# somanshu25/GPU-Accelerated-Point-Cloud-Registration-Using-Hierarchical-GMM

Hardware: AMD Instinct MI355X
Metric: EM iterations/sec (N points x J components); E-step achieved HBM GB/s (higher is better)
Workload: dtype f32; 1 GPU; BASELINE configs[2]/[4]: uniform [0,1)^3 cloud, N=1,000,000 pts per GPU (seed=rank), flat diag GMM J=800 (flavour W), fused device-resident EM, tol=0; N>1: frames are shards of one joint fit, all-reduce of (7J+2) f64 sufficient statistics per iteration; points_per_gpu=1000000, components=800, cov_type=diag, device= (gfx950:sramecc+:xnack-), compute_units=256

## Files before the change

### gpu-accelerated-point-cloud-registration-using-hierarchical-gmm_amd/csrc/flat_fused_body.h

```cpp
    constexpr int K = NSLOT;
    constexpr int KP = K / 2;
    constexpr bool ODD = (K & 1) != 0;
    const int lane = lane_id();
    f2 mu0[KP + 1], mu1[KP + 1], mu2[KP + 1], g0[KP + 1], g1[KP + 1], g2[KP + 1], cc[KP + 1];
    f2 s0[KP + 1], a0[KP + 1], a1[KP + 1], a2[KP + 1], b0[KP + 1], b1[KP + 1], b2[KP + 1];
    float mu0s = 0.f, mu1s = 0.f, mu2s = 0.f, g0s = 0.f, g1s = 0.f, g2s = 0.f, cs = NEG_INF;
    float s0s = 0.f, a0s = 0.f, a1s = 0.f, a2s = 0.f, b0s = 0.f, b1s = 0.f, b2s = 0.f;
#pragma unroll
    for (int p = 0; p < KP; ++p) {
        const int ja = (2 * p) * 64 + lane, jb = (2 * p + 1) * 64 + lane;
        mu0[p] = f2{pack[(PK_MU + 0) * Jpad + ja], pack[(PK_MU + 0) * Jpad + jb]};
        mu1[p] = f2{pack[(PK_MU + 1) * Jpad + ja], pack[(PK_MU + 1) * Jpad + jb]};
        mu2[p] = f2{pack[(PK_MU + 2) * Jpad + ja], pack[(PK_MU + 2) * Jpad + jb]};
        g0[p] = f2{pack[(PK_G + 0) * Jpad + ja], pack[(PK_G + 0) * Jpad + jb]};
        g1[p] = f2{pack[(PK_G + 1) * Jpad + ja], pack[(PK_G + 1) * Jpad + jb]};
        g2[p] = f2{pack[(PK_G + 2) * Jpad + ja], pack[(PK_G + 2) * Jpad + jb]};
        cc[p] = f2{pack[PK_C * Jpad + ja], pack[PK_C * Jpad + jb]};
        s0[p] = a0[p] = a1[p] = a2[p] = b0[p] = b1[p] = b2[p] = f2{0.f, 0.f};
    }
    if (ODD) {
        const int j = (K - 1) * 64 + lane;
        mu0s = pack[(PK_MU + 0) * Jpad + j]; mu1s = pack[(PK_MU + 1) * Jpad + j]; mu2s = pack[(PK_MU + 2) * Jpad + j];
        g0s = pack[(PK_G + 0) * Jpad + j]; g1s = pack[(PK_G + 1) * Jpad + j]; g2s = pack[(PK_G + 2) * Jpad + j];
        cs = pack[PK_C * Jpad + j];
    }

    float m0 = cs;
#pragma unroll
    for (int p = 0; p < KP; ++p) m0 = fmaxf(m0, fmaxf(cc[p].x, cc[p].y));
    m0 = wave_max_dpp(m0);
    const bool small_shift = allow_const_shift && m0 <= CS_MAX_SHIFT && m0 >= -64.0f;

    int64_t r0;
    int nrows;
    FLAT_FUSED_ROW_RANGE(n, r0, nrows);
    const float* const xw = X + 3 * r0;
    double lsum = 0.0;
    float o0 = 0.f, o1 = 0.f, o2 = 0.f, ow = 0.f;
#pragma unroll
    for (int p = 0; p < KP; ++p) {
        const float wa = pack[PK_W * Jpad + (2 * p) * 64 + lane], wb = pack[PK_W * Jpad + (2 * p + 1) * 64 + lane];
        o0 = fmaf(wa, mu0[p].x, fmaf(wb, mu0[p].y, o0));
        o1 = fmaf(wa, mu1[p].x, fmaf(wb, mu1[p].y, o1));
        o2 = fmaf(wa, mu2[p].x, fmaf(wb, mu2[p].y, o2));
        ow += wa + wb;
    }
    if (ODD) {
        const float ws = pack[PK_W * Jpad + (K - 1) * 64 + lane];
        o0 = fmaf(ws, mu0s, o0); o1 = fmaf(ws, mu1s, o1); o2 = fmaf(ws, mu2s, o2);
        ow += ws;
    }
    {
        ow = wave_sum_dpp(ow);
        const float inv_w = ow > 0.f ? 1.0f / ow : 0.f;
        o0 = wave_sum_dpp(o0) * inv_w; o1 = wave_sum_dpp(o1) * inv_w; o2 = wave_sum_dpp(o2) * inv_w;
        if (!(fabsf(o0) < 3.0e38f)) o0 = 0.f;
        if (!(fabsf(o1) < 3.0e38f)) o1 = 0.f;
        if (!(fabsf(o2) < 3.0e38f)) o2 = 0.f;
    }
    auto rows = [&](auto cs_tag) {
    constexpr bool CS = decltype(cs_tag)::value;
    if (CS) {
        const f2 M0 = f2{m0, m0};
#pragma unroll
        for (int p = 0; p < KP; ++p) cc[p] = cc[p] - M0;
        cs -= m0;
    }
    const float eps_scale = __builtin_amdgcn_exp2f(-m0);
    float eps_v = FLAT_EPS;
    asm volatile("" : "+v"(eps_v));
    float lacc = 0.f;
    float x0 = 0.f, x1 = 0.f, x2 = 0.f;
    float sw = 1.f;
    double swsum = 0.0;
    if (nrows > 0) { x0 = xw[0]; x1 = xw[1]; x2 = xw[2]; if (WEIGHTED) sw = SW[r0]; }
    for (int row = 0; row < nrows; ++row) {
        const int nrow = (row + 1 < nrows) ? row + 1 : row;
        const float* xn = xw + 3 * (int64_t)nrow;
        const float nx0 = xn[0], nx1 = xn[1], nx2 = xn[2];
        float nsw = 1.f;
        if constexpr (WEIGHTED) nsw = SW[r0 + nrow];
        if (!WEIGHTED || !weight_is_zero(sw)) {
            const f2 X0 = f2{x0, x0}, X1 = f2{x1, x1}, X2 = f2{x2, x2};
            const float xo0 = x0 - o0, xo1 = x1 - o1, xo2 = x2 - o2;
            const f2 XO0 = f2{xo0, xo0}, XO1 = f2{xo1, xo1}, XO2 = f2{xo2, xo2};

            f2 wl[KP + 1];
            f2 q0[KP + 1], q1[KP + 1], q2[KP + 1];
            float q0s = 0.f, q1s = 0.f, q2s = 0.f;
            float wls = NEG_INF;
            float m = NEG_INF;
            f2 sacc = f2{0.f, 0.f};
#pragma unroll
            for (int p = 0; p < KP; ++p) {
                const f2 d0 = X0 - mu0[p], d1 = X1 - mu1[p], d2 = X2 - mu2[p];
                q0[p] = d0 * d0; q1[p] = d1 * d1; q2[p] = d2 * d2;
                f2 a = cc[p] - g0[p] * q0[p];
                a = a - g1[p] * q1[p];
                a = a - g2[p] * q2[p];
                if (CS) {
                    wl[p] = f2{__builtin_amdgcn_exp2f(a.x), __builtin_amdgcn_exp2f(a.y)};
                    sacc = p == 0 ? wl[p] : sacc + wl[p];
                } else {
                    wl[p] = a;
                    m = fmaxf(m, fmaxf(a.x, a.y));
                }
            }
            if (ODD) {
                const float d0 = x0 - mu0s, d1 = x1 - mu1s, d2 = x2 - mu2s;
                q0s = d0 * d0; q1s = d1 * d1; q2s = d2 * d2;
                float a = fmaf(-g0s, q0s, cs);
                a = fmaf(-g1s, q1s, a);
                a = fmaf(-g2s, q2s, a);
                wls = CS ? __builtin_amdgcn_exp2f(a) : a;
                m = fmaxf(m, a);
            }
            if (CS) {
                m = m0;
            } else {
                m = wave_max_dpp(m);
                if (m == NEG_INF) m = 0.f;
                const f2 M = f2{m, m};
#pragma unroll
                for (int p = 0; p < KP; ++p) {
                    const f2 t = wl[p] - M;
                    wl[p] = f2{__builtin_amdgcn_exp2f(t.x), __builtin_amdgcn_exp2f(t.y)};
                    sacc = p == 0 ? wl[p] : sacc + wl[p];
                }
                if (ODD) wls = __builtin_amdgcn_exp2f(wls - m);
            }
            float s = sacc.x + sacc.y;
            if (ODD) s += wls;
            s = wave_sum_dpp(s);
            float inv_den;
            if (CS) {
                const float den = fmaf(eps_v, eps_scale, s);
                inv_den = __builtin_amdgcn_rcpf(den);
                if constexpr (WEIGHTED) lacc = fmaf(sw, __builtin_amdgcn_logf(den), lacc);
                else lacc += __builtin_amdgcn_logf(den);
                if constexpr (!WEIGHTED) {
                    if ((row & 7) == 7) {
                        asm volatile("" ::: "memory");
                        lsum += (double)lacc;
                        lacc = 0.f;
                    }
                }
            } else {
                const float lpn2 = lpn2_from(m, s, inv_den);
                if constexpr (WEIGHTED) lsum += (double)sw * (double)(lpn2 * LN2);
                else lsum += (double)(lpn2 * LN2);
            }
            if constexpr (WEIGHTED) inv_den *= sw;
            const f2 INV = f2{inv_den, inv_den};
#pragma unroll
            for (int p = 0; p < KP; ++p) {
                const f2 rr = wl[p] * INV;
                s0[p] += rr;
                a0[p] += rr * XO0; a1[p] += rr * XO1; a2[p] += rr * XO2;
                b0[p] += rr * q0[p]; b1[p] += rr * q1[p]; b2[p] += rr * q2[p];
            }
            if (ODD) {
                const float rr = wls * inv_den;
                s0s += rr;
                a0s = fmaf(rr, xo0, a0s); a1s = fmaf(rr, xo1, a1s); a2s = fmaf(rr, xo2, a2s);
                b0s = fmaf(rr, q0s, b0s); b1s = fmaf(rr, q1s, b1s); b2s = fmaf(rr, q2s, b2s);
            }
        }
        if constexpr (WEIGHTED) {
            if (CS && (row & 7) == 7) {
                asm volatile("" ::: "memory");
                lsum += (double)lacc;
                lacc = 0.f;
            }
        }
        x0 = nx0; x1 = nx1; x2 = nx2;
        if constexpr (WEIGHTED) sw = nsw;
    }
    if constexpr (WEIGHTED) {
        if (CS) {
            for (int64_t i = r0 + lane; i < r0 + nrows; i += 64) swsum += (double)SW[i];
            swsum = wave_sum_f64(swsum);
        }
    }
    if (CS) lsum = (lsum + (double)lacc + (WEIGHTED ? swsum : (double)nrows) * (double)m0) * (double)LN2;
    };
    if (small_shift) rows(std::true_type{});
    else rows(std::false_type{});
    {
        const f2 O0 = f2{o0, o0}, O1 = f2{o1, o1}, O2 = f2{o2, o2};
#pragma unroll
        for (int p = 0; p < KP; ++p) {
            a0[p] -= (mu0[p] - O0) * s0[p]; a1[p] -= (mu1[p] - O1) * s0[p]; a2[p] -= (mu2[p] - O2) * s0[p];
        }
        if (ODD) {
            a0s = fmaf(-(mu0s - o0), s0s, a0s); a1s = fmaf(-(mu1s - o1), s0s, a1s); a2s = fmaf(-(mu2s - o2), s0s, a2s);
        }
    }

    constexpr int ST = NSLOT * 64, STP = ST + 8, CP = FLAT_NSTAT * STP;
    __shared__ float sh[3 * CP];
    __shared__ double shl[WAVES_PER_BLOCK];
    const int w = wave_in_block();
    if (lane == 0) shl[w] = lsum;
    auto put = [&](float* base, int k, bool first, float v0, float v1, float v2, float v3, float v4, float v5, float v6) {
        float* q = base + k * 64 + lane;
        if (first) { q[0 * STP] = v0; q[1 * STP] = v1; q[2 * STP] = v2; q[3 * STP] = v3; q[4 * STP] = v4; q[5 * STP] = v5; q[6 * STP] = v6; }
        else { q[0 * STP] += v0; q[1 * STP] += v1; q[2 * STP] += v2; q[3 * STP] += v3; q[4 * STP] += v4; q[5 * STP] += v5; q[6 * STP] += v6; }
    };
    auto put_all = [&](float* base, bool first) {
#pragma unroll
        for (int p = 0; p < KP; ++p) {
            put(base, 2 * p, first, s0[p].x, a0[p].x, a1[p].x, a2[p].x, b0[p].x, b1[p].x, b2[p].x);
            put(base, 2 * p + 1, first, s0[p].y, a0[p].y, a1[p].y, a2[p].y, b0[p].y, b1[p].y, b2[p].y);
        }
        if (ODD) put(base, K - 1, first, s0s, a0s, a1s, a2s, b0s, b1s, b2s);
    };
    if (w != 1) put_all(sh + (w == 0 ? 0 : w - 1) * CP, true);
    __syncthreads();
    if (w == 1) put_all(sh, false);
    __syncthreads();
    auto total = [&](int i) { return (sh[i] + sh[CP + i]) + sh[2 * CP + i]; };
    if (comp_major) {
        float* outp = partials + (size_t)FLAT_FUSED_BLOCK * FLAT_CM_STRIDE * Jpad;
        for (int idx = threadIdx.x; idx < FLAT_CM_STRIDE * ST; idx += BLOCK) {
            const int j = idx / FLAT_CM_STRIDE, st = idx % FLAT_CM_STRIDE;
            outp[idx] = st < FLAT_NSTAT ? total(st * STP + j) : 0.f;
        }
    } else {
        float* outp = partials + (size_t)FLAT_FUSED_BLOCK * FLAT_NSTAT * Jpad;
        for (int idx = threadIdx.x; idx < FLAT_NSTAT * ST; idx += BLOCK) {
            const int st = idx / ST, j = idx % ST;
            outp[st * Jpad + j] = total(st * STP + j);
        }
    }
    if (threadIdx.x == 0) {
        double t = 0.0;
        for (int i = 0; i < WAVES_PER_BLOCK; ++i) t += shl[i];
        lpn_partials[FLAT_FUSED_BLOCK] = t;
    }
```

### gpu-accelerated-point-cloud-registration-using-hierarchical-gmm_amd/csrc/flat_fused_device.h

```cpp
#pragma once
#include "hgmm_ctx.h"
#include "wave_ops.h"

namespace hgmm {

constexpr float NEG_INF = -__builtin_huge_valf();
constexpr float LOG2E = 1.4426950408889634f;
constexpr float LN2 = 0.6931471805599453f;
constexpr int PK_MU = 0, PK_G = 3, PK_C = 6, PK_W = 7;
constexpr int PK_ROWS = 8;
typedef float f2 __attribute__((ext_vector_type(2)));
constexpr int WAVES_PER_BLOCK = 4;
constexpr int BLOCK = WAVES_PER_BLOCK * 64;

constexpr float CS_MAX_SHIFT = 60.0f;
__device__ __forceinline__ float lpn2_from(float m2, float s, float& inv_den) {
    const bool tiny = m2 < -64.0f;
    const float mc = tiny ? -64.0f : m2;
    const float den = fmaf(FLAT_EPS, __builtin_amdgcn_exp2f(-mc), tiny ? 0.0f : s);
    inv_den = tiny ? 0.0f : __builtin_amdgcn_rcpf(den);
    return mc + __builtin_amdgcn_logf(den);
}

__device__ __forceinline__ void wave_row_range(int64_t n, int64_t& r0, int64_t& r1) {
    const int64_t nw = (int64_t)gridDim.x * WAVES_PER_BLOCK;
    const int64_t gw = (int64_t)blockIdx.x * WAVES_PER_BLOCK + wave_in_block();
    const int64_t per = (n + nw - 1) / nw;
    r0 = gw * per;
    r1 = r0 + per < n ? r0 + per : n;
    if (r0 > n) r0 = n;
}
__device__ __forceinline__ int64_t uniform_i64(int64_t v) {
    const int lo = __builtin_amdgcn_readfirstlane((int)(v & 0xffffffffLL)), hi = __builtin_amdgcn_readfirstlane((int)(v >> 32));
    return ((int64_t)hi << 32) | (int64_t)(unsigned int)lo;
}
__device__ __forceinline__ void wave_row_range_uniform(int64_t n, int64_t& r0, int& nrows) {
    int64_t r1;
    wave_row_range(n, r0, r1);
    r0 = uniform_i64(r0);
    nrows = (int)(uniform_i64(r1) - r0);
}

__device__ __forceinline__ void wave_row_range_uniform(int64_t n, unsigned block, unsigned nblocks, int64_t& r0, int& nrows) {
    const int64_t nw = (int64_t)nblocks * WAVES_PER_BLOCK;
    const int64_t gw = (int64_t)block * WAVES_PER_BLOCK + wave_in_block();
    const int64_t per = (n + nw - 1) / nw;
    int64_t a = gw * per;
    const int64_t b = a + per < n ? a + per : n;
    if (a > n) a = n;
    r0 = uniform_i64(a);
    nrows = (int)(uniform_i64(b) - r0);
}

__device__ __forceinline__ bool weight_is_zero(float s) { return (__float_as_uint(s) & 0x7fffffffu) == 0u; }


template <class T>
__device__ __forceinline__ T* global_ptr(T* p) {
    typedef __attribute__((address_space(1))) T* gptr;
    return (T*)(gptr)(uintptr_t)p;
}
template <class T>
__device__ __forceinline__ const T* constant_ptr(const T* p) {
    typedef __attribute__((address_space(4))) const T* cptr;
    return (const T*)(cptr)(uintptr_t)p;
}


void launch_fused_batch_weighted(int slots, unsigned grid, hipStream_t stream, const FlatBatchMember* members,
                                 const int2* wg_table, int J, int Jpad, int parity);

}
```

Before: 3131 EM it/s (1M-pt x 800-comp frames x iterations per second, all GPUs).

## Unroll fused E-step row loop into double-buffered trips with batched point prefetch

Restructures the per-wave row loop in the fused EM kernel. For slot counts up to 13 in the small-shift path, rows are processed in trips of eight, split into two halves whose point coordinates are prefetched as a batch and held in scalar registers, with sched_barriers fencing the loads. The log-likelihood flush to double happens once per trip instead of through a per-row branch. The aim is to hide point-load latency and cut per-row loop and branch overhead, at the cost of higher register pressure, code size and a remainder loop.

```diff
diff --git a/gpu-accelerated-point-cloud-registration-using-hierarchical-gmm_amd/csrc/flat_fused_body.h b/gpu-accelerated-point-cloud-registration-using-hierarchical-gmm_amd/csrc/flat_fused_body.h
--- a/gpu-accelerated-point-cloud-registration-using-hierarchical-gmm_amd/csrc/flat_fused_body.h
+++ b/gpu-accelerated-point-cloud-registration-using-hierarchical-gmm_amd/csrc/flat_fused_body.h
@@ -70,16 +70,8 @@
     float eps_v = FLAT_EPS;
     asm volatile("" : "+v"(eps_v));
     float lacc = 0.f;
-    float x0 = 0.f, x1 = 0.f, x2 = 0.f;
-    float sw = 1.f;
     double swsum = 0.0;
-    if (nrows > 0) { x0 = xw[0]; x1 = xw[1]; x2 = xw[2]; if (WEIGHTED) sw = SW[r0]; }
-    for (int row = 0; row < nrows; ++row) {
-        const int nrow = (row + 1 < nrows) ? row + 1 : row;
-        const float* xn = xw + 3 * (int64_t)nrow;
-        const float nx0 = xn[0], nx1 = xn[1], nx2 = xn[2];
-        float nsw = 1.f;
-        if constexpr (WEIGHTED) nsw = SW[r0 + nrow];
+    auto row_em = [&](const float x0, const float x1, const float x2, const float sw) __attribute__((always_inline)) {
         if (!WEIGHTED || !weight_is_zero(sw)) {
             const f2 X0 = f2{x0, x0}, X1 = f2{x1, x1}, X2 = f2{x2, x2};
             const float xo0 = x0 - o0, xo1 = x1 - o1, xo2 = x2 - o2;
@@ -138,13 +130,6 @@
                 inv_den = __builtin_amdgcn_rcpf(den);
                 if constexpr (WEIGHTED) lacc = fmaf(sw, __builtin_amdgcn_logf(den), lacc);
                 else lacc += __builtin_amdgcn_logf(den);
-                if constexpr (!WEIGHTED) {
-                    if ((row & 7) == 7) {
-                        asm volatile("" ::: "memory");
-                        lsum += (double)lacc;
-                        lacc = 0.f;
-                    }
-                }
             } else {
                 const float lpn2 = lpn2_from(m, s, inv_den);
                 if constexpr (WEIGHTED) lsum += (double)sw * (double)(lpn2 * LN2);
@@ -161,17 +146,77 @@
             }
             if (ODD) {
                 const float rr = wls * inv_den;
-                s0s += rr;
+                if constexpr (WEIGHTED) s0s += rr;
+                else s0s = fmaf(wls, inv_den, s0s);
                 a0s = fmaf(rr, xo0, a0s); a1s = fmaf(rr, xo1, a1s); a2s = fmaf(rr, xo2, a2s);
                 b0s = fmaf(rr, q0s, b0s); b1s = fmaf(rr, q1s, b1s); b2s = fmaf(rr, q2s, b2s);
             }
         }
-        if constexpr (WEIGHTED) {
-            if (CS && (row & 7) == 7) {
-                asm volatile("" ::: "memory");
-                lsum += (double)lacc;
-                lacc = 0.f;
-            }
+    };
+    constexpr int TRIP = NSLOT <= 13 ? FUSED_TRIP : 1;
+    int row = 0;
+    if constexpr (CS && TRIP > 1) {
+        constexpr int HALF = TRIP > 1 ? TRIP / 2 : 1;
+        static_assert(8 % TRIP == 0, "a flush every eight rows falls at the end of a trip");
+        if (nrows >= TRIP) {
+            float xa[3 * HALF], xb[3 * HALF], wa[HALF], wb[HALF];
+            auto half_trip = [&](const float (&have)[3 * HALF], const float (&whave)[HALF], float (&into)[3 * HALF],
+                                 float (&winto)[HALF], const int next) __attribute__((always_inline)) {
+#pragma unroll
+                for (int t = 0; t < HALF; ++t) {
+                    float c0 = have[3 * t], c1 = have[3 * t + 1], c2 = have[3 * t + 2];
+                    asm volatile("" : "+s"(c0), "+s"(c1), "+s"(c2));
+                    row_em(c0, c1, c2, whave[t]);
+                    if (ODD) asm volatile("" : : "v"(s0s), "v"(a0s), "v"(a1s), "v"(a2s), "v"(b0s), "v"(b1s), "v"(b2s));
+                    __builtin_amdgcn_sched_barrier(0);
+                    if (t == 0) {
+                        const float* xn = xw + 3 * (int64_t)next;
+#pragma unroll
+                        for (int i = 0; i < 3 * HALF; ++i) into[i] = xn[i];
+                        if constexpr (WEIGHTED) {
+#pragma unroll
+                            for (int i = 0; i < HALF; ++i) winto[i] = SW[r0 + next + i];
+                        }
+                        __builtin_amdgcn_sched_barrier(0);
+                    }
+                }
+            };
+#pragma unroll
+            for (int i = 0; i < 3 * HALF; ++i) xa[i] = xw[i];
+#pragma unroll
+            for (int i = 0; i < HALF; ++i) wa[i] = wb[i] = 1.f;
+            if constexpr (WEIGHTED) {
+#pragma unroll
+                for (int i = 0; i < HALF; ++i) wa[i] = SW[r0 + i];
+            }
+            for (; nrows - row >= TRIP; row += TRIP) {
+                half_trip(xa, wa, xb, wb, row + HALF);
+                half_trip(xb, wb, xa, wa, nrows - row >= 2 * TRIP ? row + TRIP : row);
+                if (TRIP == 8 || ((row + TRIP) & 7) == 0) {
+                    lsum += (double)lacc;
+                    lacc = 0.f;
+                }
+            }
+        }
+    }
+    float x0 = 0.f, x1 = 0.f, x2 = 0.f;
+    float sw = 1.f;
+    if (row < nrows) {
+        const float* xr = xw + 3 * (int64_t)row;
+        x0 = xr[0]; x1 = xr[1]; x2 = xr[2];
+        if (WEIGHTED) sw = SW[r0 + row];
+    }
+    for (; row < nrows; ++row) {
+        const int nrow = (row + 1 < nrows) ? row + 1 : row;
+        const float* xn = xw + 3 * (int64_t)nrow;
+        const float nx0 = xn[0], nx1 = xn[1], nx2 = xn[2];
+        float nsw = 1.f;
+        if constexpr (WEIGHTED) nsw = SW[r0 + nrow];
+        row_em(x0, x1, x2, sw);
+        if (CS && TRIP != 8 && (row & 7) == 7) {
+            asm volatile("" ::: "memory");
+            lsum += (double)lacc;
+            lacc = 0.f;
         }
         x0 = nx0; x1 = nx1; x2 = nx2;
         if constexpr (WEIGHTED) sw = nsw;
diff --git a/gpu-accelerated-point-cloud-registration-using-hierarchical-gmm_amd/csrc/flat_fused_device.h b/gpu-accelerated-point-cloud-registration-using-hierarchical-gmm_amd/csrc/flat_fused_device.h
--- a/gpu-accelerated-point-cloud-registration-using-hierarchical-gmm_amd/csrc/flat_fused_device.h
+++ b/gpu-accelerated-point-cloud-registration-using-hierarchical-gmm_amd/csrc/flat_fused_device.h
@@ -12,6 +12,7 @@
 typedef float f2 __attribute__((ext_vector_type(2)));
 constexpr int WAVES_PER_BLOCK = 4;
 constexpr int BLOCK = WAVES_PER_BLOCK * 64;
+constexpr int FUSED_TRIP = 8;
 
 constexpr float CS_MAX_SHIFT = 60.0f;
 __device__ __forceinline__ float lpn2_from(float m2, float s, float& inv_den) {
```

After: 3267 EM it/s (1M-pt x 800-comp frames x iterations per second, all GPUs) (median of 6 runs). +4.3%, better.
